# ysymyth/3D-SDN

Hardware: AMD Instinct MI355X
Metric: rendered-objects/sec (FFD decode + transform + silhouette/normal/depth @384, fwd+bwd) (higher is better)
Workload: dtype f32

## Files before the change

3d-sdn_amd/csrc/raster_bwd.hip:

```cpp
#include "raster_math.h"
#include "sdn_common.h"

namespace sdn {

#ifndef SDN_EDGE_CHUNK
#define SDN_EDGE_CHUNK 8
#endif
constexpr int CHUNK = SDN_EDGE_CHUNK;
static_assert(CHUNK == 4 || CHUNK == 8, "k_edge_scan_sil / k_chunk_sum are written for 4 or 8");

struct BwdParams {
    const float* faces;
    const float* textures;
    const float* face_inv;
    const int32_t* face_index_map;
    const float* weight_map;
    const float* depth_map;
    const float* rgb_map;
    const float* g_rgb_out;
    const float* g_alpha_out;
    const float* g_depth_out;
    float* grad_faces;
    float* grad_textures;
    uint32_t* visible;
    int32_t* chunk_base;
    uint32_t* counter;
    uint4* chunk_desc;
    float2* chunk_out;
    const float* hmap;
    const float* hmapT;
    const uint16_t* nz_cnt;
    const uint16_t* nz_pos;
    const float* nz_val;
    uint32_t* row_cnt;
    struct OwnerRec* own_rec;
    float2* own_out;
    uint8_t* chunk_mask;
    uint32_t cap;
    double eps;
    int ts, bs, nf, S, flags;
    VertexSink sink;
};

__host__ __device__ __forceinline__ bool segment_path(const BwdParams& P)
{
#ifdef SDN_LAB_EDGE_PER_FACE
    return false;
#else
    return P.sink.grad_verts != nullptr && P.nz_cnt != nullptr;
#endif
}

struct OwnerRec {
    float t1, t0, cross;
    uint32_t kk;
    uint32_t slot;
};

struct MapReader {
    const BwdParams& P;
    int b, S, R;
    bool aa;
    __device__ MapReader(const BwdParams& p, int bn) : P(p), b(bn), S(p.S)
    {
        aa = (p.flags & SDN_AA) != 0;
        R = aa ? S / 2 : S;
    }
    __device__ __forceinline__ size_t q(int x, int y) const { return ((size_t)b * S + y) * S + x; }
    __device__ __forceinline__ int fidx(int x, int y) const { return P.face_index_map[q(x, y)]; }
    __device__ __forceinline__ float alpha(int x, int y) const { return fidx(x, y) >= 0 ? 1.0f : 0.0f; }
    __device__ __forceinline__ float rgb(int x, int y, int k) const { return P.rgb_map[q(x, y) * 3 + k]; }
    __device__ __forceinline__ size_t oidx(int x, int y) const
    {
        return aa ? ((size_t)((S - 1 - y) >> 1)) * R + (x >> 1) : ((size_t)(S - 1 - y)) * R + x;
    }
    __device__ __forceinline__ float g_alpha(int x, int y) const
    {
        if (!P.g_alpha_out) return 0.0f;
        const float g = P.g_alpha_out[(size_t)b * R * R + oidx(x, y)];
        return aa ? g * 0.25f : g;
    }
    __device__ __forceinline__ float g_depth(int x, int y) const
    {
        if (!P.g_depth_out) return 0.0f;
        const float g = P.g_depth_out[(size_t)b * R * R + oidx(x, y)];
        return aa ? g * 0.25f : g;
    }
    __device__ __forceinline__ float g_rgb(int x, int y, int k) const
    {
        if (!P.g_rgb_out) return 0.0f;
        const float g = P.g_rgb_out[((size_t)b * 3 + k) * R * R + oidx(x, y)];
        return aa ? g * 0.25f : g;
    }
};

__device__ __forceinline__ float edge_dist(float pa, float pb, float denom, int d1, float d1_cross, float is_f,
                                           double eps)
{
    float t = (pb - pa) / denom;
    t = t * ((float)d1 - d1_cross);
    float dist = (2.0f * t) / is_f;
    dist = (0.0f < dist) ? (float)((double)dist + eps) : (float)((double)dist - eps);
    return dist;
}

struct EdgeWalk {
    float p[3][2];
    int pi0, pi1;
    int direction;
    int d0_from, d0_to;
};

__device__ __forceinline__ EdgeWalk edge_walk(const float face[9], int edge_num, int axis, float is_f)
{
    EdgeWalk w;
    int pi[3];
    float pp[3][2];
#pragma unroll
    for (int num = 0; num < 3; num++) {
        pi[num] = (edge_num + num) % 3;
        pp[num][0] = ndc_to_pixel(face[3 * pi[num] + 0], is_f);
        pp[num][1] = ndc_to_pixel(face[3 * pi[num] + 1], is_f);
    }
#pragma unroll
    for (int num = 0; num < 3; num++) {
        w.p[num][0] = pp[num][axis];
        w.p[num][1] = pp[num][1 - axis];
    }
    w.pi0 = pi[0];
    w.pi1 = pi[1];
    if (axis == 0)
        w.direction = (w.p[0][0] < w.p[1][0]) ? -1 : 1;
    else
        w.direction = (w.p[0][0] < w.p[1][0]) ? 1 : -1;
    w.d0_from = cvt_i32(fmaxf(ceilf(fminf(w.p[0][0], w.p[1][0])), 0.0f));
    w.d0_to = cvt_i32(fminf(fmaxf(w.p[0][0], w.p[1][0]), is_f - 1.0f));
    return w;
}

__device__ __forceinline__ void edge_pixel(const BwdParams& P, const MapReader& M, const EdgeWalk& w, int fn, int axis,
                                           int d0, bool use_alpha, bool use_rgb, int lane, int nlanes, float& acc0,
                                           float& acc1)
{
    const int S = P.S;
    const float is_f = (float)S;
    const float fd0 = (float)d0;
    float d1_cross = (w.p[1][1] - w.p[0][1]) / (w.p[1][0] - w.p[0][0]);
    d1_cross = d1_cross * (fd0 - w.p[0][0]);
    d1_cross = d1_cross + w.p[0][1];
    const int d1_in = (0 < w.direction) ? cvt_i32(floorf(d1_cross)) : cvt_i32(ceilf(d1_cross));
    const int d1_out = d1_in + w.direction;
    if (d1_in < 0 || S <= d1_in) return;
    if (d1_out < 0 || S <= d1_out) return;

    const int xin = axis == 0 ? d0 : d1_in, yin = axis == 0 ? d1_in : d0;
    const int xout = axis == 0 ? d0 : d1_out, yout = axis == 0 ? d1_out : d0;
    float alpha_in = 0.f, alpha_out = 0.f, rgb_in[3] = {0, 0, 0}, rgb_out[3] = {0, 0, 0};
    const int f_in = M.fidx(xin, yin);
    if (use_alpha) {
        alpha_in = f_in >= 0 ? 1.0f : 0.0f;
        alpha_out = M.alpha(xout, yout);
    }
    if (use_rgb) {
#pragma unroll
        for (int k = 0; k < 3; k++) {
            rgb_in[k] = M.rgb(xin, yin, k);
            rgb_out[k] = M.rgb(xout, yout, k);
        }
    }
    const bool nz1 = w.p[1][0] != fd0, nz0 = w.p[0][0] != fd0;
    const float den1 = w.p[1][0] - fd0, den0 = fd0 - w.p[0][0];
    const float* hline = nullptr;
    if (P.hmap && use_alpha && !use_rgb) hline = (axis == 0 ? P.hmapT : P.hmap) + ((size_t)M.b * S + d0) * S;

    if (f_in == fn && hline) {
        const int d1_limit = (0 < w.direction) ? S - 1 : 0;
        const int d1_from = max(min(d1_out, d1_limit), 0);
        const int d1_to = min(max(d1_out, d1_limit), S - 1);
        const size_t row = (size_t)(axis == 0 ? P.bs : 0) * S + (size_t)M.b * S + d0;
        const uint16_t* cnt = P.nz_cnt + row * (S + 1);
        const int k1 = cnt[d1_to + 1];
        for (int k = cnt[d1_from] + lane; k < k1; k += nlanes) {
            const int d1 = P.nz_pos[row * S + k];
            const float diff_grad = P.nz_val[row * S + k];
            if (nz1) acc0 -= diff_grad / edge_dist(w.p[0][0], w.p[1][0], den1, d1, d1_cross, is_f, P.eps);
            if (nz0) acc1 -= diff_grad / edge_dist(w.p[0][0], w.p[1][0], den0, d1, d1_cross, is_f, P.eps);
        }
    } else if (f_in == fn) {
        const int d1_limit = (0 < w.direction) ? S - 1 : 0;
        const int d1_from = max(min(d1_out, d1_limit), 0);
        const int d1_to = min(max(d1_out, d1_limit), S - 1);
        for (int d1 = d1_from + lane; d1 <= d1_to; d1 += nlanes) {
            const int x = axis == 0 ? d0 : d1, y = axis == 0 ? d1 : d0;
            float diff_grad = 0.0f;
            if (use_alpha) diff_grad = diff_grad + (M.alpha(x, y) - alpha_in) * M.g_alpha(x, y);
            if (use_rgb) {
#pragma unroll
                for (int k = 0; k < 3; k++) diff_grad = diff_grad + (M.rgb(x, y, k) - rgb_in[k]) * M.g_rgb(x, y, k);
            }
            if (diff_grad <= 0) continue;
            if (nz1) acc0 -= diff_grad / edge_dist(w.p[0][0], w.p[1][0], den1, d1, d1_cross, is_f, P.eps);
            if (nz0) acc1 -= diff_grad / edge_dist(w.p[0][0], w.p[1][0], den0, d1, d1_cross, is_f, P.eps);
        }
    }
    {
        float d0_cross2;
        if ((fd0 - w.p[0][0]) * (fd0 - w.p[2][0]) < 0) {
            d0_cross2 = (w.p[2][1] - w.p[0][1]) / (w.p[2][0] - w.p[0][0]);
            d0_cross2 = d0_cross2 * (fd0 - w.p[0][0]);
            d0_cross2 = d0_cross2 + w.p[0][1];
        } else {
            d0_cross2 = (w.p[1][1] - w.p[2][1]) / (w.p[1][0] - w.p[2][0]);
            d0_cross2 = d0_cross2 * (fd0 - w.p[2][0]);
            d0_cross2 = d0_cross2 + w.p[2][1];
        }
        const int d1_limit = (0 < w.direction) ? cvt_i32(ceilf(d0_cross2)) : cvt_i32(floorf(d0_cross2));
        const int d1_from = max(min(d1_in, d1_limit), 0);
        const int d1_to = min(max(d1_in, d1_limit), S - 1);
        for (int d1 = d1_from + lane; d1 <= d1_to; d1 += nlanes) {
            const int x = axis == 0 ? d0 : d1, y = axis == 0 ? d1 : d0;
            if (M.fidx(x, y) != fn) continue;
            float diff_grad = 0.0f;
            if (use_alpha) diff_grad = diff_grad + (1.0f - alpha_out) * M.g_alpha(x, y);
            if (use_rgb) {
#pragma unroll
                for (int k = 0; k < 3; k++) diff_grad = diff_grad + (M.rgb(x, y, k) - rgb_out[k]) * M.g_rgb(x, y, k);
            }
            if (diff_grad <= 0) continue;
            if (nz1) acc0 -= diff_grad / edge_dist(w.p[0][0], w.p[1][0], den1, d1, d1_cross, is_f, P.eps);
            if (nz0) acc1 -= diff_grad / edge_dist(w.p[0][0], w.p[1][0], den0, d1, d1_cross, is_f, P.eps);
        }
    }
}

__global__ __launch_bounds__(256) void k_mark_visible(const int32_t* __restrict__ face_index_map, long npx, int S,
                                                       int nf, uint32_t* __restrict__ visible)
{
    const long i = (long)blockIdx.x * 256 + threadIdx.x;
    if (i >= npx) return;
    const int fn = face_index_map[i];
    if (fn >= 0) visible[(i / ((long)S * S)) * nf + fn] = 1u;
}

__global__ __launch_bounds__(256) void k_hmap(const BwdParams P, float* __restrict__ hmapT)
{
    __shared__ float tile[32][33];
    const int S = P.S, b = blockIdx.z;
    const MapReader M(P, b);
    const int x = blockIdx.x * 32 + (threadIdx.x & 31);
#pragma unroll
    for (int r = 0; r < 4; r++) {
        const int ly = (threadIdx.x >> 5) + 8 * r, y = blockIdx.y * 32 + ly;
        float h = 0.0f;
        if (x < S && y < S) {
            const int fn = M.fidx(x, y);
            if (fn < 0) {
                const float t = (0.0f - 1.0f) * M.g_alpha(x, y);
                h = t > 0.0f ? t : 0.0f;
            } else {
                P.visible[(size_t)b * P.nf + fn] = 1u;
            }
        }
        tile[ly][threadIdx.x & 31] = h;
    }
    __syncthreads();
    const int yt = blockIdx.y * 32 + (threadIdx.x & 31);
#pragma unroll
    for (int r = 0; r < 4; r++) {
        const int lx = (threadIdx.x >> 5) + 8 * r, xt = blockIdx.x * 32 + lx;
        if (xt < S && yt < S) hmapT[((size_t)b * S + xt) * S + yt] = tile[threadIdx.x & 31][lx];
    }
}

__global__ __launch_bounds__(256) void k_compact_rows(const BwdParams P, const float* __restrict__ mapsT,
                                                      size_t rows_per_map, int S, uint16_t* __restrict__ cnt,
                                                      uint16_t* __restrict__ pos, float* __restrict__ val)
{
    const int lane = threadIdx.x & 63;
    const size_t row = (size_t)blockIdx.x * 4 + (threadIdx.x >> 6);
    if (row >= 2 * rows_per_map) return;
    const bool image_row = row < rows_per_map;
    const float* src = mapsT + (image_row ? 0 : row - rows_per_map) * S;
    const int yb = (int)(row / (size_t)S), yy = (int)(row % (size_t)S);
    const MapReader M(P, image_row ? yb : 0);
    auto h_at = [&](const int x) {
        float h = 0.0f;
        if (M.fidx(x, yy) < 0) {
            const float t = (0.0f - 1.0f) * M.g_alpha(x, yy);
            h = t > 0.0f ? t : 0.0f;
        }
        return h;
    };
    uint16_t* c = cnt + row * (S + 1);
    int base = 0;
    for (int x0 = 0; x0 < S; x0 += 128) {
        const int x = x0 + 2 * lane;
        float h0 = 0.0f, h1 = 0.0f;
        if (image_row) {
            if (x < S) h0 = h_at(x);
            if (x + 1 < S) h1 = h_at(x + 1);
        } else if (x + 1 < S && ((S & 1) == 0)) {
            const float2 v = *reinterpret_cast<const float2*>(src + x);
            h0 = v.x;
            h1 = v.y;
        } else {
            if (x < S) h0 = src[x];
            if (x + 1 < S) h1 = src[x + 1];
        }
        const bool nz0 = h0 > 0.0f, nz1 = h1 > 0.0f;
        const unsigned long long m0 = __ballot(nz0), m1 = __ballot(nz1);
        const unsigned long long below = (1ull << lane) - 1ull;
        const int i0 = base + __popcll(m0 & below) + __popcll(m1 & below);
        const int i1 = i0 + (nz0 ? 1 : 0);
        if (x < S) {
            c[x] = (uint16_t)i0;
            if (nz0) {
                pos[row * S + i0] = (uint16_t)x;
                val[row * S + i0] = h0;
            }
        }
        if (x + 1 < S) {
            c[x + 1] = (uint16_t)i1;
            if (nz1) {
                pos[row * S + i1] = (uint16_t)(x + 1);
                val[row * S + i1] = h1;
            }
        }
        base += __popcll(m0) + __popcll(m1);
    }
    if (lane == 0) c[S] = (uint16_t)base;
}

constexpr int PLAN_THREADS = 1024;
__global__ __launch_bounds__(PLAN_THREADS) void k_edge_plan(const BwdParams P)
{
    const long i = (long)blockIdx.x * PLAN_THREADS + threadIdx.x;
    const long total = (long)P.bs * P.nf;
    if (P.sink.grad_verts) {
        const long n = (long)P.bs * P.sink.nv * 3;
        for (long k = i; k < n; k += (long)gridDim.x * PLAN_THREADS) P.sink.grad_verts[k] = 0.0f;
    }
    const int lane = threadIdx.x & 63;
    int from[6], cnt[6];
    uint32_t nchunks = 0;
    bool contributes = false;
    if (i < total) {
        const bool active = (P.flags & (SDN_ALPHA | SDN_RGB)) != 0;
        if (active && P.visible[i] != 0u) {
            float face[9];
#pragma unroll
            for (int k = 0; k < 9; k++) face[k] = P.faces[i * 9 + k];
            if (!is_backface(face)) {
                const float is_f = (float)P.S;
#pragma unroll
                for (int e = 0; e < 6; e++) {
                    const EdgeWalk w = edge_walk(face, e >> 1, e & 1, is_f);
                    from[e] = w.d0_from;
                    cnt[e] = max(w.d0_to - w.d0_from + 1, 0);
                    nchunks += (uint32_t)((cnt[e] + CHUNK - 1) / CHUNK);
                }
                contributes = nchunks != 0;
            }
        }
    }
    __shared__ uint32_t wave_sum[PLAN_THREADS / 64];
    __shared__ uint32_t block_base;
    uint32_t incl = nchunks;
#pragma unroll
    for (int d = 1; d < 64; d <<= 1) {
        const uint32_t o = __shfl_up(incl, d, 64);
        if (lane >= d) incl += o;
    }
    const int wave = threadIdx.x >> 6;
    if (lane == 63) wave_sum[wave] = incl;
    __syncthreads();
    if (threadIdx.x == 0) {
        uint32_t tot = 0;
        for (int w = 0; w < PLAN_THREADS / 64; w++) tot += wave_sum[w];
        block_base = tot ? atomicAdd(P.counter, tot) : 0u;
    }
    __syncthreads();
    uint32_t wave_base = block_base;
    for (int w = 0; w < wave; w++) wave_base += wave_sum[w];
    if (i >= total) return;
    const bool per_face = !segment_path(P);
    if (!contributes) {
        if (per_face) P.chunk_base[i] = -2;
        return;
    }
    const uint32_t base = wave_base + incl - nchunks;
    if (base + nchunks > P.cap) {
        if (per_face)
            P.chunk_base[i] = -1;
        else
            P.chunk_base[atomicAdd(P.counter + 1, 1u)] = (int32_t)i;
        for (uint32_t c = base; c < P.cap; c++) P.chunk_desc[c] = make_uint4(0xffffffffu, 0xffffffffu, 0u, 0u);
        return;
    }
    if (per_face) P.chunk_base[i] = (int32_t)base;
    uint32_t c = base;
#pragma unroll
    for (int e = 0; e < 6; e++) {
        for (int s = 0; s < cnt[e]; s += CHUNK)
            P.chunk_desc[c++] = make_uint4((uint32_t)i, (uint32_t)e, (uint32_t)(from[e] + s),
                                           (uint32_t)min(CHUNK, cnt[e] - s));
    }
}

__global__ __launch_bounds__(256) void k_edge_scan(const BwdParams P)
{
    const int lane = threadIdx.x & 63;
    const uint32_t wave = (blockIdx.x * 256u + threadIdx.x) >> 6;
    const uint32_t nwaves = (gridDim.x * 256u) >> 6;
    const uint32_t nchunks = min(*P.counter, P.cap);
    const bool use_alpha = (P.flags & SDN_ALPHA) != 0;
    const bool use_rgb = (P.flags & SDN_RGB) != 0;
    const float is_f = (float)P.S;
    for (uint32_t c = wave; c < nchunks; c += nwaves) {
        const uint4 d = P.chunk_desc[c];
        if (d.x >= (uint32_t)((long)P.bs * P.nf)) {
            if (lane == 0) P.chunk_out[c] = make_float2(0.f, 0.f);
            continue;
        }
        const long i = d.x;
        const int bn = (int)(i / P.nf), fn = (int)(i % P.nf);
        float face[9];
#pragma unroll
        for (int k = 0; k < 9; k++) face[k] = P.faces[i * 9 + k];
        const int axis = (int)(d.y & 1u);
        const EdgeWalk w = edge_walk(face, (int)(d.y >> 1), axis, is_f);
        const MapReader M(P, bn);
        float acc0 = 0.f, acc1 = 0.f;
        for (int s = 0; s < (int)d.w; s++)
            edge_pixel(P, M, w, fn, axis, (int)d.z + s, use_alpha, use_rgb, lane, 64, acc0, acc1);
#pragma unroll
        for (int o = 32; o > 0; o >>= 1) {
            acc0 += __shfl_xor(acc0, o, 64);
            acc1 += __shfl_xor(acc1, o, 64);
        }
        if (lane == 0) P.chunk_out[c] = make_float2(acc0, acc1);
    }
}

#ifndef SDN_LAB_IN_LANE_MAX
#define SDN_LAB_IN_LANE_MAX 32
#endif
constexpr int IN_LANE_MAX = SDN_LAB_IN_LANE_MAX;
#ifndef SDN_LAB_COOP_MAX_WALKS
#define SDN_LAB_COOP_MAX_WALKS 32
#endif
constexpr int COOP_MAX_WALKS = SDN_LAB_COOP_MAX_WALKS;

__global__ __launch_bounds__(256) void k_edge_scan_sil(const BwdParams P)
{
    const int lane = threadIdx.x & 63;
    const uint32_t wave = (blockIdx.x * 256u + threadIdx.x) >> 6;
    const uint32_t nwaves = (gridDim.x * 256u) >> 6;
    const uint32_t nchunks = min(*P.counter, P.cap);
    const int S = P.S;
    const float is_f = (float)S;
    const float two_over_is = 2.0f / is_f, eps_f = (float)P.eps;
    const long total_faces = (long)P.bs * P.nf;
    constexpr uint32_t CPW = 64u / CHUNK;
    for (uint32_t c0 = wave * CPW; c0 < nchunks; c0 += nwaves * CPW) {
        const uint32_t c = c0 + (uint32_t)(lane / CHUNK);
        const int s_in = lane % CHUNK;
        float in0 = 0.f, in1 = 0.f;
        int k0 = 0, k1 = 0;
        bool up = false;
        size_t row = 0;
        float pa = 0.f, pb = 0.f, den1 = 1.f, den0 = 1.f, d1_cross = 0.f;
        int nzflags = 0;
        bool chunk_ok = false;
        int w_from = 0, w_to = -1, w_key = 0, w_d0 = 0;
        float w_ta1 = 0.f, w_ta0 = 0.f;
        if (c < nchunks) {
            const uint4 d = P.chunk_desc[c];
            chunk_ok = d.x < (uint32_t)total_faces;
            if (chunk_ok && s_in < (int)d.w) {
                const long i = d.x;
                const int bn = (int)(i / P.nf), fn = (int)(i % P.nf);
                float face[9];
#pragma unroll
                for (int k = 0; k < 9; k++) face[k] = P.faces[i * 9 + k];
                const int axis = (int)(d.y & 1u);
                const EdgeWalk w = edge_walk(face, (int)(d.y >> 1), axis, is_f);
                const MapReader M(P, bn);
                const int d0 = (int)d.z + s_in;
                const float fd0 = (float)d0;
                d1_cross = (w.p[1][1] - w.p[0][1]) / (w.p[1][0] - w.p[0][0]);
                d1_cross = d1_cross * (fd0 - w.p[0][0]);
                d1_cross = d1_cross + w.p[0][1];
                const int d1_in = (0 < w.direction) ? cvt_i32(floorf(d1_cross)) : cvt_i32(ceilf(d1_cross));
                const int d1_out = d1_in + w.direction;
                if (!(d1_in < 0 || S <= d1_in || d1_out < 0 || S <= d1_out)) {
                    const int xin = axis == 0 ? d0 : d1_in, yin = axis == 0 ? d1_in : d0;
                    const int xout = axis == 0 ? d0 : d1_out, yout = axis == 0 ? d1_out : d0;
                    const int f_in = M.fidx(xin, yin);
                    const float alpha_out = M.alpha(xout, yout);
                    const bool nz1 = w.p[1][0] != fd0, nz0 = w.p[0][0] != fd0;
                    pa = w.p[0][0];
                    pb = w.p[1][0];
                    den1 = w.p[1][0] - fd0;
                    den0 = fd0 - w.p[0][0];
                    nzflags = (nz1 ? 1 : 0) | (nz0 ? 2 : 0);
                    if (f_in == fn) {
                        const int d1_limit = (0 < w.direction) ? S - 1 : 0;
                        const int d1_from = max(min(d1_out, d1_limit), 0);
                        const int d1_to = min(max(d1_out, d1_limit), S - 1);
                        row = (size_t)(axis == 0 ? P.bs : 0) * S + (size_t)bn * S + d0;
                        const uint16_t* cnt = P.nz_cnt + row * (S + 1);
                        up = 0 < w.direction;
                        if (up) {
                            k0 = cnt[d1_from];
                            k1 = cnt[S];
                        } else {
                            k0 = 0;
                            k1 = cnt[d1_to + 1];
                        }
                    }
#ifdef SDN_LAB_SCAN_NOIN
                    if (false) {
#else
                    if (alpha_out == 0.0f) {
#endif
                    float d0_cross2;
                    if ((fd0 - w.p[0][0]) * (fd0 - w.p[2][0]) < 0) {
                        d0_cross2 = (w.p[2][1] - w.p[0][1]) / (w.p[2][0] - w.p[0][0]);
                        d0_cross2 = d0_cross2 * (fd0 - w.p[0][0]);
                        d0_cross2 = d0_cross2 + w.p[0][1];
                    } else {
                        d0_cross2 = (w.p[1][1] - w.p[2][1]) / (w.p[1][0] - w.p[2][0]);
                        d0_cross2 = d0_cross2 * (fd0 - w.p[2][0]);
                        d0_cross2 = d0_cross2 + w.p[2][1];
                    }
                    const int d1_limit = (0 < w.direction) ? cvt_i32(ceilf(d0_cross2)) : cvt_i32(floorf(d0_cross2));
                    const int d1_from = max(min(d1_in, d1_limit), 0);
                    const int d1_to = min(max(d1_in, d1_limit), S - 1);
                    const float ta1 = (pb - pa) / den1 * two_over_is, ta0 = (pb - pa) / den0 * two_over_is;
                    w_from = d1_from;
                    w_to = d1_to;
                    w_key = axis | (fn << 1);
                    w_d0 = d0 | (bn << 16);
                    w_ta1 = ta1;
                    w_ta0 = ta0;
                    }
                }
            }
        }
        {
            const bool has = w_to >= w_from;
            unsigned long long lm = __ballot(has && w_to - w_from >= IN_LANE_MAX);
            const bool coop = __popcll(lm) <= COOP_MAX_WALKS;
            if (!coop) lm = 0ull;
            const bool own = has && (coop ? w_to - w_from < IN_LANE_MAX : true);
            while (lm) {
                const int j = __builtin_amdgcn_readfirstlane(__ffsll((long long)lm) - 1);
                lm &= lm - 1ull;
                const int from = __builtin_amdgcn_readlane(w_from, j), to = __builtin_amdgcn_readlane(w_to, j);
                const int key = __builtin_amdgcn_readlane(w_key, j), d0b = __builtin_amdgcn_readlane(w_d0, j);
                const float ta1 = __int_as_float(__builtin_amdgcn_readlane(__float_as_int(w_ta1), j));
                const float ta0 = __int_as_float(__builtin_amdgcn_readlane(__float_as_int(w_ta0), j));
                const float cross = __int_as_float(__builtin_amdgcn_readlane(__float_as_int(d1_cross), j));
                const int nzj = __builtin_amdgcn_readlane(nzflags, j);
                const int axis = key & 1, fn = key >> 1, d0 = d0b & 0xffff;
                const MapReader M(P, d0b >> 16);
                float p0 = 0.f, p1 = 0.f;
                for (int d1 = from + lane; d1 <= to; d1 += 64) {
                    const int x = axis == 0 ? d0 : d1, y = axis == 0 ? d1 : d0;
                    if (M.fidx(x, y) != fn) continue;
                    float diff_grad = 0.0f;
                    diff_grad = diff_grad + (1.0f - 0.0f) * M.g_alpha(x, y);
                    if (diff_grad <= 0) continue;
                    const float dd = (float)d1 - cross;
                    if (nzj & 1) {
                        const float dist = ta1 * dd;
                        p0 -= diff_grad * __builtin_amdgcn_rcpf(0.0f < dist ? dist + eps_f : dist - eps_f);
                    }
                    if (nzj & 2) {
                        const float dist = ta0 * dd;
                        p1 -= diff_grad * __builtin_amdgcn_rcpf(0.0f < dist ? dist + eps_f : dist - eps_f);
                    }
                }
#pragma unroll
                for (int o = 32; o > 0; o >>= 1) {
                    p0 += __shfl_xor(p0, o, 64);
                    p1 += __shfl_xor(p1, o, 64);
                }
                if (lane == j) {
                    in0 += p0;
                    in1 += p1;
                }
            }
            if (own) {
                const int axis = w_key & 1, fn = w_key >> 1, d0 = w_d0 & 0xffff;
                const MapReader M(P, w_d0 >> 16);
                const bool nz1 = (nzflags & 1) != 0, nz0 = (nzflags & 2) != 0;
                for (int d1b = w_from; d1b <= w_to; d1b += 4) {
                    int fi[4];
                    float ga[4];
#pragma unroll
                    for (int u = 0; u < 4; u++) {
                        const int d1 = min(d1b + u, w_to);
                        const int x = axis == 0 ? d0 : d1, y = axis == 0 ? d1 : d0;
                        fi[u] = M.fidx(x, y);
                        ga[u] = M.g_alpha(x, y);
                    }
#pragma unroll
                    for (int u = 0; u < 4; u++) {
                        const int d1 = d1b + u;
                        if (d1 > w_to || fi[u] != fn) continue;
                        float diff_grad = 0.0f;
                        diff_grad = diff_grad + (1.0f - 0.0f) * ga[u];
                        if (diff_grad <= 0) continue;
                        const float dd = (float)d1 - d1_cross;
                        if (nz1) {
                            const float dist = w_ta1 * dd;
                            in0 -= diff_grad * __builtin_amdgcn_rcpf(0.0f < dist ? dist + eps_f : dist - eps_f);
                        }
                        if (nz0) {
                            const float dist = w_ta0 * dd;
                            in1 -= diff_grad * __builtin_amdgcn_rcpf(0.0f < dist ? dist + eps_f : dist - eps_f);
                        }
                    }
                }
            }
        }
#ifdef SDN_LAB_SCAN_NOFILE
        const bool owner = false;
#else
        const bool owner = k1 > k0;
#endif
        if (owner) {
            uint32_t at = atomicAdd(P.row_cnt + 2 * row + (up ? 0 : 1), 1u);
            if (!up) at = (uint32_t)(3 * S) - 1u - at;
            OwnerRec r;
            r.t1 = (pb - pa) / den1 * two_over_is;
            r.t0 = (pb - pa) / den0 * two_over_is;
            r.cross = d1_cross;
            r.kk = (uint32_t)k0 | ((uint32_t)k1 << 16);
            r.slot = (c * (uint32_t)CHUNK + (uint32_t)s_in) | ((uint32_t)nzflags << 30);
            if (at < (uint32_t)(3 * S)) P.own_rec[row * (size_t)(3 * S) + at] = r;
        }
        const unsigned long long owners = __ballot(owner);
        float sum0 = in0, sum1 = in1;
#pragma unroll
        for (int o = CHUNK / 2; o > 0; o >>= 1) {
            const float t0 = __shfl_down(sum0, o, 64), t1 = __shfl_down(sum1, o, 64);
            if (s_in + o < CHUNK) {
                sum0 += t0;
                sum1 += t1;
            }
        }
        if (s_in == 0 && c < nchunks) {
            P.chunk_out[c] = chunk_ok ? make_float2(sum0, sum1) : make_float2(0.f, 0.f);
            P.chunk_mask[c] = chunk_ok ? (uint8_t)((owners >> (lane & ~(CHUNK - 1))) & ((1ull << CHUNK) - 1ull)) : (uint8_t)0;
        }
    }
}

__global__ __launch_bounds__(256) void k_edge_rows(const BwdParams P, int nrows)
{
    extern __shared__ float2 lds_list[];
    const int lane = threadIdx.x & 63, wave = threadIdx.x >> 6;
    const int S = P.S;
    const int row = blockIdx.x;
    const float eps_f = (float)P.eps;
    const uint32_t n_up = min(P.row_cnt[2 * row], (uint32_t)(3 * S));
    const uint32_t n_down = min(P.row_cnt[2 * row + 1], (uint32_t)(3 * S) - n_up);
    if (n_up + n_down == 0) return;
    const int total = P.nz_cnt[(size_t)row * (S + 1) + S];
    for (int k = threadIdx.x; k < total; k += 256)
        lds_list[k] = make_float2((float)P.nz_pos[(size_t)row * S + k], P.nz_val[(size_t)row * S + k]);
    __syncthreads();
    const OwnerRec* recs = P.own_rec + (size_t)row * (3 * S);
    const uint32_t b_up = (n_up + 63) >> 6, b_all = b_up + ((n_down + 63) >> 6);
    for (uint32_t b = wave; b < b_all; b += 4) {
        const bool down = b >= b_up;
        const uint32_t idx = (down ? b - b_up : b) * 64u + lane;
        if (idx >= (down ? n_down : n_up)) continue;
        const OwnerRec r = recs[down ? (uint32_t)(3 * S) - 1u - idx : idx];
        const int k0 = (int)(r.kk & 0xffffu), k1 = (int)(r.kk >> 16);
        const bool nz1 = (r.slot >> 30) & 1u, nz0 = (r.slot >> 31) & 1u;
        typedef float v2f __attribute__((ext_vector_type(2)));
        const v2f t = {r.t1, r.t0};
        const float sdd = down ? -1.0f : 1.0f;
        const v2f es = {0.0f < t.x * sdd ? eps_f : -eps_f, 0.0f < t.y * sdd ? eps_f : -eps_f};
        v2f o[4] = {{0.f, 0.f}, {0.f, 0.f}, {0.f, 0.f}, {0.f, 0.f}};
        auto term = [&](const float2 e, v2f& a) {
            float val = e.y;
#ifndef SDN_LAB_ROWS_HI_SPLAT
            asm volatile("" : "+v"(val));
#endif
            const float dd = e.x - r.cross;
            v2f dist = t * dd;
#ifdef SDN_LAB_ROWS_EPS_PER_ENTRY
            const v2f s = {0.0f < dist.x ? eps_f : -eps_f, 0.0f < dist.y ? eps_f : -eps_f};
            dist = dist + s;
#else
            dist = dist + es;
#endif
            const v2f rc = {__builtin_amdgcn_rcpf(dist.x), __builtin_amdgcn_rcpf(dist.y)};
            a = a - val * rc;
        };
        int k = k0;
        for (; k + 4 <= k1; k += 4) {
            const float2 e0 = lds_list[k], e1 = lds_list[k + 1], e2 = lds_list[k + 2], e3 = lds_list[k + 3];
            term(e0, o[0]);
            term(e1, o[1]);
            term(e2, o[2]);
            term(e3, o[3]);
        }
        if (k < k1) term(lds_list[k], o[0]);
        if (k + 1 < k1) term(lds_list[k + 1], o[1]);
        if (k + 2 < k1) term(lds_list[k + 2], o[2]);
        const v2f sum = (o[0] + o[1]) + (o[2] + o[3]);
        P.own_out[r.slot & 0x3fffffffu] = make_float2(nz1 ? sum.x : 0.0f, nz0 ? sum.y : 0.0f);
    }
}

__device__ __forceinline__ float2 chunk_add_owners(const BwdParams& P, uint32_t c, uint32_t m, float2 a)
{
    const float4* q = reinterpret_cast<const float4*>(P.own_out + (size_t)c * CHUNK);
#pragma unroll
    for (int h = 0; h < CHUNK / 2; h++) {
        if (!(m & (3u << (2 * h)))) continue;
        const float4 v = q[h];
        if (m & (1u << (2 * h))) {
            a.x += v.x;
            a.y += v.y;
        }
        if (m & (2u << (2 * h))) {
            a.x += v.z;
            a.y += v.w;
        }
    }
    return a;
}

__global__ __launch_bounds__(256) void k_chunk_sum(const BwdParams P)
{
    const uint32_t nchunks = min(*P.counter, P.cap);
    const uint32_t c = blockIdx.x * 256u + threadIdx.x;
    if (c >= nchunks) return;
    uint32_t m = P.chunk_mask[c];
    if (!m) return;
    P.chunk_out[c] = chunk_add_owners(P, c, m, P.chunk_out[c]);
}

__device__ __forceinline__ void sink_add_face(const BwdParams& P, long i, const float grad_face[9])
{
    bool any = false;
#pragma unroll
    for (int k = 0; k < 9; k++) any = any || grad_face[k] != 0.0f;
    if (!any) return;
    const int bn = (int)(i / P.nf), fn = (int)(i % P.nf);
    const bool twin = P.sink.fill_back && fn >= P.sink.nf0;
    const int32_t* idx = P.sink.faces_idx + (size_t)bn * P.sink.fstride + (size_t)(twin ? fn - P.sink.nf0 : fn) * 3;
#pragma unroll
    for (int k = 0; k < 3; k++) {
        float* dst = P.sink.grad_verts + ((size_t)bn * P.sink.nv + idx[twin ? 2 - k : k]) * 3;
#pragma unroll
        for (int d = 0; d < 3; d++)
            if (grad_face[3 * k + d] != 0.0f) unsafeAtomicAdd(&dst[d], grad_face[3 * k + d]);
    }
}

__global__ __launch_bounds__(256) void k_edge_reduce(const BwdParams P)
{
    const long i = (long)blockIdx.x * 256 + threadIdx.x;
    const long total = (long)P.bs * P.nf;
    if (i >= total) return;
    const bool accumulate = (P.flags & SDN_ACCUMULATE) != 0;
    if ((P.flags & SDN_SPARSE_GRAD) && P.visible[i] == 0u) return;
    const int32_t base = P.chunk_base[i];
    float grad_face[9] = {0, 0, 0, 0, 0, 0, 0, 0, 0};
    if (base != -2) {
        float face[9];
#pragma unroll
        for (int k = 0; k < 9; k++) face[k] = P.faces[i * 9 + k];
        const float is_f = (float)P.S;
        const bool use_alpha = (P.flags & SDN_ALPHA) != 0;
        const bool use_rgb = (P.flags & SDN_RGB) != 0;
        const int bn = (int)(i / P.nf), fn = (int)(i % P.nf);
        uint32_t c = (uint32_t)base;
        for (int e = 0; e < 6; e++) {
            const int axis = e & 1;
            const EdgeWalk w = edge_walk(face, e >> 1, axis, is_f);
            float a0 = 0.f, a1 = 0.f;
            if (base >= 0) {
                const int cnt = max(w.d0_to - w.d0_from + 1, 0);
                const int nch = (cnt + CHUNK - 1) / CHUNK;
                for (int s = 0; s < nch; s += 8) {
                    float2 o[8];
#pragma unroll
                    for (int u = 0; u < 8; u++)
                        if (s + u < nch) o[u] = P.chunk_out[c + s + u];
#pragma unroll
                    for (int u = 0; u < 8; u++)
                        if (s + u < nch) {
                            a0 += o[u].x;
                            a1 += o[u].y;
                        }
                }
                c += (uint32_t)nch;
                grad_face[w.pi0 * 3 + (1 - axis)] += a0;
                grad_face[w.pi1 * 3 + (1 - axis)] += a1;
            } else {
                const MapReader M(P, bn);
                for (int d0 = w.d0_from; d0 <= w.d0_to; d0++)
                    edge_pixel(P, M, w, fn, axis, d0, use_alpha, use_rgb, 0, 1, grad_face[w.pi0 * 3 + (1 - axis)],
                               grad_face[w.pi1 * 3 + (1 - axis)]);
            }
        }
    }
    if (P.sink.grad_verts) {
        if (base == -2) return;
        sink_add_face(P, i, grad_face);
        return;
    }
    if (accumulate) {
#pragma unroll
        for (int k = 0; k < 9; k++) P.grad_faces[i * 9 + k] += grad_face[k];
    } else {
#pragma unroll
        for (int k = 0; k < 9; k++) P.grad_faces[i * 9 + k] = grad_face[k];
    }
}

constexpr int SEG_SERIAL_BLOCKS = 8;

__device__ __forceinline__ void segment_add(const BwdParams& P, long i, int e, float a0, float a1)
{
    if (a0 == 0.0f && a1 == 0.0f) return;
    const int bn = (int)(i / P.nf), fn = (int)(i % P.nf);
    const int axis = e & 1, pi0 = e >> 1, pi1 = (pi0 + 1) % 3;
    const bool twin = P.sink.fill_back && fn >= P.sink.nf0;
    const int32_t* idx = P.sink.faces_idx + (size_t)bn * P.sink.fstride + (size_t)(twin ? fn - P.sink.nf0 : fn) * 3;
    float* g = P.sink.grad_verts + (size_t)bn * P.sink.nv * 3 + (1 - axis);
    if (a0 != 0.0f) unsafeAtomicAdd(&g[(size_t)idx[twin ? 2 - pi0 : pi0] * 3], a0);
    if (a1 != 0.0f) unsafeAtomicAdd(&g[(size_t)idx[twin ? 2 - pi1 : pi1] * 3], a1);
}

__global__ __launch_bounds__(256) void k_edge_segments(const BwdParams P)
{
    const int lane = threadIdx.x & 63;
    if (blockIdx.x < SEG_SERIAL_BLOCKS) {
        const uint32_t n = P.counter[1];
        constexpr uint32_t WAVES = SEG_SERIAL_BLOCKS * 4;
        const uint32_t wave = blockIdx.x * 4u + (threadIdx.x >> 6);
        const bool use_alpha = (P.flags & SDN_ALPHA) != 0, use_rgb = (P.flags & SDN_RGB) != 0;
        const float is_f = (float)P.S;
        for (uint32_t k = (uint32_t)lane * WAVES + wave; k < n; k += 64u * WAVES) {
            const long i = P.chunk_base[k];
            const int bn = (int)(i / P.nf), fn = (int)(i % P.nf);
            float face[9];
#pragma unroll
            for (int j = 0; j < 9; j++) face[j] = P.faces[i * 9 + j];
            const MapReader M(P, bn);
            float grad_face[9] = {0, 0, 0, 0, 0, 0, 0, 0, 0};
            for (int e = 0; e < 6; e++) {
                const int axis = e & 1;
                const EdgeWalk w = edge_walk(face, e >> 1, axis, is_f);
                for (int d0 = w.d0_from; d0 <= w.d0_to; d0++)
                    edge_pixel(P, M, w, fn, axis, d0, use_alpha, use_rgb, 0, 1, grad_face[w.pi0 * 3 + (1 - axis)],
                               grad_face[w.pi1 * 3 + (1 - axis)]);
            }
            sink_add_face(P, i, grad_face);
        }
        return;
    }
    const uint32_t nchunks = min(*P.counter, P.cap);
    const uint32_t c = (blockIdx.x - (uint32_t)SEG_SERIAL_BLOCKS) * 256u + threadIdx.x;
    const uint32_t c_wave = (uint32_t)__builtin_amdgcn_readfirstlane((int)(c - (uint32_t)lane));
    if (c_wave >= nchunks) return;
    const uint32_t total = (uint32_t)((long)P.bs * P.nf);
    auto key_at = [&](uint32_t s) { return *reinterpret_cast<const uint2*>(P.chunk_desc + s); };
    uint2 d = make_uint2(0xffffffffu, 0xffffffffu);
    float2 v = make_float2(0.f, 0.f);
    uint32_t m = 0u;
    if (c < nchunks) {
        d = key_at(c);
        v = P.chunk_out[c];
        m = P.chunk_mask[c];
    }
    uint2 before = make_uint2(0xffffffffu, 0xffffffffu), after = before;
    if (c_wave > 0u) before = key_at(c_wave - 1u);
    if (c_wave + 64u < nchunks) after = key_at(c_wave + 64u);
    const bool valid = d.x < total;
    if (valid && m) v = chunk_add_owners(P, c, m, v);
    uint32_t px = __shfl_up(d.x, 1, 64), py = __shfl_up(d.y, 1, 64);
    if (lane == 0) {
        px = before.x;
        py = before.y;
    }
    const bool head = valid && (px != d.x || py != d.y);
    const unsigned long long bounds = __ballot(head || !valid);
    const unsigned long long above = lane == 63 ? 0ull : bounds >> (lane + 1);
    const int len = head ? (above ? __ffsll((long long)above) : 64 - lane) : 0;
    float a0 = 0.f, a1 = 0.f;
    for (int k = 0; __ballot(k < len) != 0ull; k++) {
        const float tx = __shfl(v.x, lane + k, 64), ty = __shfl(v.y, lane + k, 64);
        if (k < len) {
            a0 += tx;
            a1 += ty;
        }
    }
    const unsigned long long runs_on = __ballot(head && !above && after.x == d.x && after.y == d.y);
    if (runs_on) {
        const int hl = __ffsll((long long)runs_on) - 1;
        const uint32_t kx = (uint32_t)__builtin_amdgcn_readlane((int)d.x, hl), ky = (uint32_t)__builtin_amdgcn_readlane((int)d.y, hl);
        for (uint32_t s0 = c_wave + 64u; s0 < nchunks; s0 += 64u) {
            const uint32_t s = s0 + (uint32_t)lane;
            uint2 ds = make_uint2(0xffffffffu, 0xffffffffu);
            float2 vs = make_float2(0.f, 0.f);
            uint32_t ms = 0u;
            if (s < nchunks) {
                ds = key_at(s);
                vs = P.chunk_out[s];
                ms = P.chunk_mask[s];
            }
            const bool mine = ds.x == kx && ds.y == ky;
            if (mine && ms) vs = chunk_add_owners(P, s, ms, vs);
            const unsigned long long others = ~__ballot(mine);
            const int n = others ? __ffsll((long long)others) - 1 : 64;
            for (int k = 0; k < n; k++) {
                const float tx = __shfl(vs.x, k, 64), ty = __shfl(vs.y, k, 64);
                if (lane == hl) {
                    a0 += tx;
                    a1 += ty;
                }
            }
            if (n < 64) break;
        }
    }
    if (!head) return;
    segment_add(P, (long)d.x, (int)d.y, a0, a1);
}

__global__ __launch_bounds__(256) void k_bwd_pixels(const BwdParams P)
{
    const long i = (long)blockIdx.x * 256 + threadIdx.x;
    const long npx = (long)P.bs * P.S * P.S;
    if (i >= npx) return;
    const int fn = P.face_index_map[i];
    if (fn < 0) return;
    const int S = P.S;
    const int bn = (int)(i / ((long)S * S));
    const int pn = (int)(i % ((long)S * S));
    const int yi = pn / S, xi = pn % S;
    const MapReader M(P, bn);
    const size_t fidx = (size_t)bn * P.nf + fn;
    float face[9];
#pragma unroll
    for (int k = 0; k < 9; k++) face[k] = P.faces[fidx * 9 + k];
    const float depth = P.depth_map[i];
    const float w[3] = {P.weight_map[i * 3 + 0], P.weight_map[i * 3 + 1], P.weight_map[i * 3 + 2]};

    if ((P.flags & SDN_DEPTH) && P.g_depth_out) {
        float inv[9];
#pragma unroll
        for (int k = 0; k < 9; k++) inv[k] = P.face_inv[fidx * 9 + k];
        const float g = M.g_depth(xi, yi);
        const float depth2 = depth * depth;
        float* gf = P.grad_faces + fidx * 9;
#pragma unroll
        for (int k = 0; k < 3; k++) {
            const float zk = face[3 * k + 2];
            float t = g * w[k];
            t = t * depth2;
            t = t / (zk * zk);
            unsafeAtomicAdd(&gf[3 * k + 2], t);
        }
        float tmp[2] = {0.f, 0.f};
#pragma unroll
        for (int k = 0; k < 2; k++)
#pragma unroll
            for (int l = 0; l < 3; l++) tmp[k] = tmp[k] + (-inv[3 * l + k] / face[3 * l + 2]);
#pragma unroll
        for (int k = 0; k < 3; k++)
#pragma unroll
            for (int l = 0; l < 2; l++) {
                float t = -g * tmp[l];
                t = t * w[k];
                t = t * depth2;
                t = t * (float)S;
                t = t / 2.0f;
                unsafeAtomicAdd(&gf[3 * k + l], t);
            }
    }
    if ((P.flags & SDN_RGB) && P.g_rgb_out && P.grad_textures) {
        const bool face_color = (P.flags & SDN_FACE_COLOR) != 0;
        const int ts = face_color ? 2 : P.ts;
        const TexCoord tc = texture_coord(w, depth, face[2], face[5], face[8], ts, P.eps);
        const float g[3] = {M.g_rgb(xi, yi, 0), M.g_rgb(xi, yi, 1), M.g_rgb(xi, yi, 2)};
        if (face_color) {
            float acc[3] = {0.f, 0.f, 0.f};
#pragma unroll
            for (int c = 0; c < 8; c++) {
                int isc;
                float wgt;
                texture_corner(tc, c, ts, isc, wgt);
#pragma unroll
                for (int k = 0; k < 3; k++) acc[k] = acc[k] + wgt * g[k];
            }
#pragma unroll
            for (int k = 0; k < 3; k++) unsafeAtomicAdd(&P.grad_textures[fidx * 3 + k], acc[k]);
        } else {
            float* gt = P.grad_textures + fidx * (size_t)ts * ts * ts * 3;
#pragma unroll
            for (int c = 0; c < 8; c++) {
                int isc;
                float wgt;
                texture_corner(tc, c, ts, isc, wgt);
#pragma unroll
                for (int k = 0; k < 3; k++) unsafeAtomicAdd(&gt[(long)isc * 3 + k], wgt * g[k]);
            }
        }
    }
}

}

using namespace sdn;

static size_t align256(size_t n) { return (n + 255) & ~(size_t)255; }

static void bwd_layout(int bs, int nf, int S, size_t off[14], uint32_t& cap, size_t& total)
{
    const size_t n = (size_t)bs * nf;
    cap = (uint32_t)(4 * n + 65536);
    off[0] = 0;
    off[1] = 256;
    off[10] = off[1] + align256(n * sizeof(uint32_t));
    off[2] = off[10] + align256((size_t)4 * bs * S * sizeof(uint32_t));
    off[3] = off[2] + align256(n * sizeof(int32_t));
    off[4] = off[3] + align256((size_t)cap * sizeof(uint4));
    off[5] = off[4] + align256((size_t)cap * sizeof(float2));
    off[6] = off[5];
    off[7] = off[6] + align256((size_t)bs * S * S * sizeof(float));
    off[8] = off[7] + align256((size_t)2 * bs * S * (S + 1) * sizeof(uint16_t));
    off[9] = off[8] + align256((size_t)2 * bs * S * S * sizeof(uint16_t));
    off[11] = off[9] + align256((size_t)2 * bs * S * S * sizeof(float));
    off[12] = off[11] + align256((size_t)2 * bs * S * 3 * S * sizeof(OwnerRec));
    off[13] = off[12] + align256((size_t)cap * 8 * sizeof(float2));
    total = off[13] + align256((size_t)cap);
}

namespace sdn {
const uint32_t* raster_bwd_visible_flags(const void* workspace) { return (const uint32_t*)((const char*)workspace + 256); }
}

SDN_API int sdn_raster_bwd_workspace_bytes(int bs, int nf, int S, size_t* out)
{
    if (bs <= 0 || nf <= 0 || S <= 0 || !out) return fail(SDN_EINVAL, "sdn_raster_bwd_workspace_bytes: bad sizes");
    size_t off[14], total;
    uint32_t cap;
    bwd_layout(bs, nf, S, off, cap, total);
    *out = total;
    return SDN_OK;
}

SDN_API int sdn_rasterize_bwd(const float* faces, const float* textures, int ts, int bs, int nf, int S, double eps,
                              int flags, const float* face_inv, const int32_t* face_index_map,
                              const float* weight_map, const float* depth_map, const float* rgb_map,
                              const float* g_rgb_out, const float* g_alpha_out, const float* g_depth_out,
                              float* grad_faces, float* grad_textures, void* workspace, size_t workspace_bytes,
                              sdnStream stream)
{
    return rasterize_bwd_core(nullptr, faces, textures, ts, bs, nf, S, eps, flags, face_inv, face_index_map, weight_map, depth_map,
                              rgb_map, g_rgb_out, g_alpha_out, g_depth_out, grad_faces, grad_textures, workspace, workspace_bytes,
                              stream);
}

int sdn::rasterize_bwd_core(const VertexSink* sink, const float* faces, const float* textures, int ts, int bs, int nf, int S,
                            double eps, int flags, const float* face_inv, const int32_t* face_index_map, const float* weight_map,
                            const float* depth_map, const float* rgb_map, const float* g_rgb_out, const float* g_alpha_out,
                            const float* g_depth_out, float* grad_faces, float* grad_textures, void* workspace,
                            size_t workspace_bytes, sdnStream stream)
{
    if (!faces || !face_inv || !face_index_map || !weight_map || !depth_map || (!grad_faces && !sink) || bs <= 0 || nf <= 0 ||
        S <= 0)
        return fail(SDN_EINVAL, "sdn_rasterize_bwd: missing state (was the forward run with SDN_SAVE_MAPS?)");
    if (sink && ((flags & (SDN_RGB | SDN_DEPTH | SDN_ACCUMULATE)) || !(flags & SDN_ALPHA) || !g_alpha_out || !sink->faces_idx ||
                 !sink->grad_verts || nf != (sink->fill_back ? 2 : 1) * sink->nf0))
        return fail(SDN_EINVAL, "rasterize_bwd_core: the vertex sink takes a silhouette-only pass");
    if ((flags & SDN_RGB) && (!rgb_map || !textures))
        return fail(SDN_EINVAL, "sdn_rasterize_bwd: rgb gradients need rgb_map and textures");
    if ((flags & SDN_AA) && (S & 1)) return fail(SDN_EINVAL, "sdn_rasterize_bwd: SDN_AA needs an even internal size");
    size_t off[14], need;
    uint32_t cap;
    bwd_layout(bs, nf, S, off, cap, need);
    if (!workspace || workspace_bytes < need)
        return fail(SDN_ENOMEM, "sdn_rasterize_bwd: workspace %zu < %zu bytes", workspace_bytes, need);
    hipStream_t st = (hipStream_t)stream;
    BwdParams P;
    P.faces = faces;
    P.textures = textures;
    P.face_inv = face_inv;
    P.face_index_map = face_index_map;
    P.weight_map = weight_map;
    P.depth_map = depth_map;
    P.rgb_map = rgb_map;
    P.g_rgb_out = (flags & SDN_RGB) ? g_rgb_out : nullptr;
    P.g_alpha_out = (flags & SDN_ALPHA) ? g_alpha_out : nullptr;
    P.g_depth_out = (flags & SDN_DEPTH) ? g_depth_out : nullptr;
    P.grad_faces = grad_faces;
    P.grad_textures = grad_textures;
    char* ws = (char*)workspace;
    P.counter = (uint32_t*)(ws + off[0]);
    P.visible = (uint32_t*)(ws + off[1]);
    P.chunk_base = (int32_t*)(ws + off[2]);
    P.chunk_desc = (uint4*)(ws + off[3]);
    P.chunk_out = (float2*)(ws + off[4]);
    P.hmap = nullptr;
    P.hmapT = nullptr;
    P.nz_cnt = nullptr;
    P.nz_pos = nullptr;
    P.nz_val = nullptr;
    P.row_cnt = nullptr;
    P.own_rec = nullptr;
    P.own_out = nullptr;
    P.chunk_mask = nullptr;
    P.cap = (flags & SDN_SERIAL_EDGES) ? 0u : cap;
    P.eps = eps;
    P.ts = ts;
    P.bs = bs;
    P.nf = nf;
    P.S = S;
    P.flags = flags;
    P.sink = sink ? *sink : VertexSink{nullptr, 0, 0, 0, 0, nullptr};
    if (!P.g_rgb_out) P.flags &= ~SDN_RGB;
    if (!P.g_alpha_out) P.flags &= ~SDN_ALPHA;
    const long total = (long)bs * nf;
    const long npx = (long)bs * S * S;
    const bool edges = (P.flags & (SDN_ALPHA | SDN_RGB)) != 0;
    if (!edges) P.flags &= ~SDN_SPARSE_GRAD;
    int rc;
    if (edges) {
        hipError_t e = hipMemsetAsync(ws, 0, off[2], st);
        if (e != hipSuccess) return fail(SDN_ELAUNCH, "hipMemsetAsync(plan): %s", hipGetErrorString(e));
        const bool sil_path = (P.flags & SDN_ALPHA) && !(P.flags & SDN_RGB) && !(flags & SDN_SERIAL_EDGES);
        if (!sil_path) {
            hipLaunchKernelGGL(k_mark_visible, dim3(cdiv(npx, 256)), dim3(256), 0, st, face_index_map, npx, S, nf,
                               P.visible);
            if ((rc = check_launch("k_mark_visible"))) return rc;
        }
        if (sil_path) {
            float* hmap = (float*)(ws + off[5]);
            float* hmapT = (float*)(ws + off[6]);
            if (S > 65535) return fail(SDN_EINVAL, "sdn_rasterize_bwd: internal size %d exceeds the 16-bit row index", S);
            uint16_t* cnt = (uint16_t*)(ws + off[7]);
            uint16_t* pos = (uint16_t*)(ws + off[8]);
            float* val = (float*)(ws + off[9]);
            const size_t rows = (size_t)bs * S;
            hipLaunchKernelGGL(k_hmap, dim3(cdiv(S, 32), cdiv(S, 32), bs), dim3(256), 0, st, P, hmapT);
            if ((rc = check_launch("k_hmap"))) return rc;
            hipLaunchKernelGGL(k_compact_rows, dim3((unsigned)cdiv((long)(2 * rows), 4)), dim3(256), 0, st, P, hmapT, rows, S, cnt, pos,
                               val);
            if ((rc = check_launch("k_compact_rows"))) return rc;
            P.hmap = hmap;
            P.hmapT = hmapT;
            P.nz_cnt = cnt;
            P.nz_pos = pos;
            P.nz_val = val;
            if ((size_t)cap * 8 >= (1u << 30)) return fail(SDN_EINVAL, "sdn_rasterize_bwd: %u chunks exceed the 30-bit slot index", cap);
            P.row_cnt = (uint32_t*)(ws + off[10]);
            P.own_rec = (OwnerRec*)(ws + off[11]);
            P.own_out = (float2*)(ws + off[12]);
            P.chunk_mask = (uint8_t*)(ws + off[13]);
        }
    }
    hipLaunchKernelGGL(k_edge_plan, dim3(cdiv(total, PLAN_THREADS)), dim3(PLAN_THREADS), 0, st, P);
    if ((rc = check_launch("k_edge_plan"))) return rc;
    if (edges) {
        {
            TimedLaunch timed(TIME_EDGE_SCAN, st, 0.0);
            if (P.nz_cnt) {
                hipLaunchKernelGGL(k_edge_scan_sil, dim3(256 * 8), dim3(256), 0, st, P);
                const int nrows = 2 * bs * S;
                hipLaunchKernelGGL(k_edge_rows, dim3((unsigned)nrows), dim3(256), (size_t)S * sizeof(float2), st, P, nrows);
                if (!segment_path(P)) hipLaunchKernelGGL(k_chunk_sum, dim3(cdiv((long)cap, 256)), dim3(256), 0, st, P);
            } else
                hipLaunchKernelGGL(k_edge_scan, dim3(256 * 8), dim3(256), 0, st, P);
        }
        if ((rc = check_launch("k_edge_scan"))) return rc;
    }
    if (segment_path(P)) {
        hipLaunchKernelGGL(k_edge_segments, dim3((unsigned)(cdiv((long)cap, 256) + SEG_SERIAL_BLOCKS)), dim3(256), 0, st, P);
        if ((rc = check_launch("k_edge_segments"))) return rc;
    } else {
        hipLaunchKernelGGL(k_edge_reduce, dim3(cdiv(total, 256)), dim3(256), 0, st, P);
        if ((rc = check_launch("k_edge_reduce"))) return rc;
    }

    const bool need_tex = (P.flags & SDN_RGB) && grad_textures;
    if (need_tex && !(flags & SDN_ACCUMULATE)) {
        const size_t n = (flags & SDN_FACE_COLOR) ? (size_t)total * 3 : (size_t)total * ts * ts * ts * 3;
        hipError_t e = hipMemsetAsync(grad_textures, 0, n * sizeof(float), st);
        if (e != hipSuccess) return fail(SDN_ELAUNCH, "hipMemsetAsync(grad_textures): %s", hipGetErrorString(e));
    }
    if (((P.flags & SDN_DEPTH) && P.g_depth_out) || need_tex) {
        hipLaunchKernelGGL(k_bwd_pixels, dim3(cdiv(npx, 256)), dim3(256), 0, st, P);
        if ((rc = check_launch("k_bwd_pixels"))) return rc;
    }
    return SDN_OK;
}
```

Before: 24550.

## Replace float hit maps with coverage bitmasks and low-res gradient transpose

```diff
diff --git a/3d-sdn_amd/csrc/raster_bwd.hip b/3d-sdn_amd/csrc/raster_bwd.hip
--- a/3d-sdn_amd/csrc/raster_bwd.hip
+++ b/3d-sdn_amd/csrc/raster_bwd.hip
@@ -27,8 +27,6 @@
     uint32_t* counter;
     uint4* chunk_desc;
     float2* chunk_out;
-    const float* hmap;
-    const float* hmapT;
     const uint16_t* nz_cnt;
     const uint16_t* nz_pos;
     const float* nz_val;
@@ -170,10 +168,9 @@
     }
     const bool nz1 = w.p[1][0] != fd0, nz0 = w.p[0][0] != fd0;
     const float den1 = w.p[1][0] - fd0, den0 = fd0 - w.p[0][0];
-    const float* hline = nullptr;
-    if (P.hmap && use_alpha && !use_rgb) hline = (axis == 0 ? P.hmapT : P.hmap) + ((size_t)M.b * S + d0) * S;
-
-    if (f_in == fn && hline) {
+    const bool sparse_rows = P.nz_cnt && use_alpha && !use_rgb;
+
+    if (f_in == fn && sparse_rows) {
         const int d1_limit = (0 < w.direction) ? S - 1 : 0;
         const int d1_from = max(min(d1_out, d1_limit), 0);
         const int d1_to = min(max(d1_out, d1_limit), S - 1);
@@ -242,37 +239,52 @@
     if (fn >= 0) visible[(i / ((long)S * S)) * nf + fn] = 1u;
 }
 
-__global__ __launch_bounds__(256) void k_hmap(const BwdParams P, float* __restrict__ hmapT)
-{
-    __shared__ float tile[32][33];
-    const int S = P.S, b = blockIdx.z;
-    const MapReader M(P, b);
-    const int x = blockIdx.x * 32 + (threadIdx.x & 31);
+__global__ __launch_bounds__(256) void k_cover_bits(const BwdParams P, uint32_t* __restrict__ cov, uint32_t* __restrict__ covT,
+                                                    float* __restrict__ gT)
+{
+    __shared__ uint32_t flag[32][33];
+    __shared__ float gt[32][33];
+    const int S = P.S, b = blockIdx.z, W = (S + 31) >> 5;
+    const bool aa = (P.flags & SDN_AA) != 0;
+    const int R = aa ? S / 2 : S, n = aa ? 16 : 32;
+    const int lx = threadIdx.x & 31, l8 = threadIdx.x >> 5;
+    const unsigned half = threadIdx.x & 32;
+    const int x = blockIdx.x * 32 + lx;
+    int fn[4];
+    float gv[4];
 #pragma unroll
     for (int r = 0; r < 4; r++) {
-        const int ly = (threadIdx.x >> 5) + 8 * r, y = blockIdx.y * 32 + ly;
-        float h = 0.0f;
-        if (x < S && y < S) {
-            const int fn = M.fidx(x, y);
-            if (fn < 0) {
-                const float t = (0.0f - 1.0f) * M.g_alpha(x, y);
-                h = t > 0.0f ? t : 0.0f;
-            } else {
-                P.visible[(size_t)b * P.nf + fn] = 1u;
-            }
-        }
-        tile[ly][threadIdx.x & 31] = h;
+        const int ly = l8 + 8 * r, y = blockIdx.y * 32 + ly;
+        const int xo = blockIdx.x * n + lx, yo = blockIdx.y * n + ly;
+        fn[r] = (x < S && y < S) ? P.face_index_map[((size_t)b * S + y) * S + x] : -1;
+        gv[r] = (lx < n && ly < n && xo < R && yo < R) ? P.g_alpha_out[((size_t)b * R + yo) * R + xo] : 0.0f;
+    }
+#pragma unroll
+    for (int r = 0; r < 4; r++) {
+        const int ly = l8 + 8 * r, y = blockIdx.y * 32 + ly;
+        const bool covered = fn[r] >= 0;
+        const int left = __shfl_up(fn[r], 1);
+        if (covered && ((threadIdx.x & 63) == 0 || left != fn[r])) P.visible[(size_t)b * P.nf + fn[r]] = 1u;
+        flag[ly][lx] = covered ? 1u : 0u;
+        gt[ly][lx] = gv[r];
+        const unsigned long long m = __ballot(covered);
+        if (lx == 0 && y < S) cov[((size_t)b * S + y) * W + blockIdx.x] = (uint32_t)(m >> half);
     }
     __syncthreads();
-    const int yt = blockIdx.y * 32 + (threadIdx.x & 31);
 #pragma unroll
     for (int r = 0; r < 4; r++) {
-        const int lx = (threadIdx.x >> 5) + 8 * r, xt = blockIdx.x * 32 + lx;
-        if (xt < S && yt < S) hmapT[((size_t)b * S + xt) * S + yt] = tile[threadIdx.x & 31][lx];
-    }
-}
-
-__global__ __launch_bounds__(256) void k_compact_rows(const BwdParams P, const float* __restrict__ mapsT,
+        const int lc = l8 + 8 * r, xt = blockIdx.x * 32 + lc;
+        const unsigned long long m = __ballot(flag[lx][lc] != 0u);
+        if (lx == 0 && xt < S) covT[((size_t)b * S + xt) * W + blockIdx.y] = (uint32_t)(m >> half);
+        const int xo = blockIdx.x * n + lc, yo = blockIdx.y * n + lx;
+        if (lx < n && lc < n && xo < R && yo < R) gT[((size_t)b * R + xo) * R + yo] = gt[lx][lc];
+    }
+}
+
+constexpr int CR = 6;
+template <bool AA>
+__global__ __launch_bounds__(256) void k_compact_rows(const BwdParams P, const uint32_t* __restrict__ cov,
+                                                      const uint32_t* __restrict__ covT, const float* __restrict__ gT,
                                                       size_t rows_per_map, int S, uint16_t* __restrict__ cnt,
                                                       uint16_t* __restrict__ pos, float* __restrict__ val)
 {
@@ -280,55 +292,75 @@
     const size_t row = (size_t)blockIdx.x * 4 + (threadIdx.x >> 6);
     if (row >= 2 * rows_per_map) return;
     const bool image_row = row < rows_per_map;
-    const float* src = mapsT + (image_row ? 0 : row - rows_per_map) * S;
-    const int yb = (int)(row / (size_t)S), yy = (int)(row % (size_t)S);
-    const MapReader M(P, image_row ? yb : 0);
-    auto h_at = [&](const int x) {
-        float h = 0.0f;
-        if (M.fidx(x, yy) < 0) {
-            const float t = (0.0f - 1.0f) * M.g_alpha(x, yy);
-            h = t > 0.0f ? t : 0.0f;
-        }
-        return h;
-    };
+    const size_t line = image_row ? row : row - rows_per_map;
+    const int b = (int)(line / (size_t)S), d0 = (int)(line % (size_t)S);
+    const int R = AA ? S / 2 : S, W = (S + 31) >> 5;
+    const uint32_t* cw = (image_row ? cov : covT) + line * W;
+    const float* gl = image_row ? P.g_alpha_out + ((size_t)b * R + (R - 1 - (AA ? d0 >> 1 : d0))) * R
+                                : gT + ((size_t)b * R + (AA ? d0 >> 1 : d0)) * R;
     uint16_t* c = cnt + row * (S + 1);
+    const bool odd = ((row * (size_t)(S + 1)) & 1) != 0;
+    const unsigned long long below = (1ull << lane) - 1ull;
     int base = 0;
-    for (int x0 = 0; x0 < S; x0 += 128) {
-        const int x = x0 + 2 * lane;
-        float h0 = 0.0f, h1 = 0.0f;
-        if (image_row) {
-            if (x < S) h0 = h_at(x);
-            if (x + 1 < S) h1 = h_at(x + 1);
-        } else if (x + 1 < S && ((S & 1) == 0)) {
-            const float2 v = *reinterpret_cast<const float2*>(src + x);
-            h0 = v.x;
-            h1 = v.y;
-        } else {
-            if (x < S) h0 = src[x];
-            if (x + 1 < S) h1 = src[x + 1];
-        }
-        const bool nz0 = h0 > 0.0f, nz1 = h1 > 0.0f;
-        const unsigned long long m0 = __ballot(nz0), m1 = __ballot(nz1);
-        const unsigned long long below = (1ull << lane) - 1ull;
-        const int i0 = base + __popcll(m0 & below) + __popcll(m1 & below);
-        const int i1 = i0 + (nz0 ? 1 : 0);
-        if (x < S) {
-            c[x] = (uint16_t)i0;
-            if (nz0) {
-                pos[row * S + i0] = (uint16_t)x;
-                val[row * S + i0] = h0;
-            }
-        }
-        if (x + 1 < S) {
-            c[x + 1] = (uint16_t)i1;
-            if (nz1) {
-                pos[row * S + i1] = (uint16_t)(x + 1);
-                val[row * S + i1] = h1;
-            }
-        }
-        base += __popcll(m0) + __popcll(m1);
-    }
-    if (lane == 0) c[S] = (uint16_t)base;
+    if (AA && odd && lane == 0) c[0] = 0;
+    for (int e0 = 0; e0 < R; e0 += 64 * CR) {
+        float g[CR];
+        uint32_t w[CR];
+#pragma unroll
+        for (int j = 0; j < CR; j++) {
+            const int e = e0 + 64 * j + lane;
+            g[j] = 0.0f;
+            w[j] = 0u;
+            if (e < R) {
+                g[j] = gl[image_row ? e : R - 1 - e];
+                w[j] = cw[AA ? e >> 4 : e >> 5];
+            }
+        }
+#pragma unroll
+        for (int j = 0; j < CR; j++) {
+            const int e = e0 + 64 * j + lane;
+            if (e0 + 64 * j >= R) break;
+            const float t = (0.0f - 1.0f) * (AA ? g[j] * 0.25f : g[j]);
+            const float h = t > 0.0f ? t : 0.0f;
+            const bool in = e < R && h > 0.0f;
+            if (AA) {
+                const uint32_t two = w[j] >> (2 * (e & 15));
+                const bool nz0 = in && !(two & 1u), nz1 = in && !(two & 2u);
+                const unsigned long long m0 = __ballot(nz0), m1 = __ballot(nz1);
+                const int i0 = base + __popcll(m0 & below) + __popcll(m1 & below);
+                const int i1 = i0 + (nz0 ? 1 : 0), i2 = i1 + (nz1 ? 1 : 0);
+                if (e < R) {
+                    const int x = 2 * e;
+                    if (odd)
+                        *reinterpret_cast<uint32_t*>(c + x + 1) = (uint32_t)i1 | (uint32_t)i2 << 16;
+                    else
+                        *reinterpret_cast<uint32_t*>(c + x) = (uint32_t)i0 | (uint32_t)i1 << 16;
+                    if (nz0) {
+                        pos[row * S + i0] = (uint16_t)x;
+                        val[row * S + i0] = h;
+                    }
+                    if (nz1) {
+                        pos[row * S + i1] = (uint16_t)(x + 1);
+                        val[row * S + i1] = h;
+                    }
+                }
+                base += __popcll(m0) + __popcll(m1);
+            } else {
+                const bool nz = in && !((w[j] >> (e & 31)) & 1u);
+                const unsigned long long m = __ballot(nz);
+                const int i0 = base + __popcll(m & below);
+                if (e < R) {
+                    c[e] = (uint16_t)i0;
+                    if (nz) {
+                        pos[row * S + i0] = (uint16_t)e;
+                        val[row * S + i0] = h;
+                    }
+                }
+                base += __popcll(m);
+            }
+        }
+    }
+    if (lane == 0 && !(AA && odd)) c[S] = (uint16_t)base;
 }
 
 constexpr int PLAN_THREADS = 1024;
@@ -1113,8 +1145,6 @@
     P.chunk_base = (int32_t*)(ws + off[2]);
     P.chunk_desc = (uint4*)(ws + off[3]);
     P.chunk_out = (float2*)(ws + off[4]);
-    P.hmap = nullptr;
-    P.hmapT = nullptr;
     P.nz_cnt = nullptr;
     P.nz_pos = nullptr;
     P.nz_val = nullptr;
@@ -1140,27 +1170,33 @@
     if (edges) {
         hipError_t e = hipMemsetAsync(ws, 0, off[2], st);
         if (e != hipSuccess) return fail(SDN_ELAUNCH, "hipMemsetAsync(plan): %s", hipGetErrorString(e));
-        const bool sil_path = (P.flags & SDN_ALPHA) && !(P.flags & SDN_RGB) && !(flags & SDN_SERIAL_EDGES);
+        const size_t cov_words = (size_t)(S + 31) / 32;
+        const bool setup_fits = 2 * (size_t)bs * S * cov_words * sizeof(uint32_t) <= off[7] - off[6] &&
+                                (size_t)bs * S * S * sizeof(float) <= off[12] - off[11];
+        const bool sil_path = (P.flags & SDN_ALPHA) && !(P.flags & SDN_RGB) && !(flags & SDN_SERIAL_EDGES) && setup_fits;
         if (!sil_path) {
             hipLaunchKernelGGL(k_mark_visible, dim3(cdiv(npx, 256)), dim3(256), 0, st, face_index_map, npx, S, nf,
                                P.visible);
             if ((rc = check_launch("k_mark_visible"))) return rc;
         }
         if (sil_path) {
-            float* hmap = (float*)(ws + off[5]);
-            float* hmapT = (float*)(ws + off[6]);
             if (S > 65535) return fail(SDN_EINVAL, "sdn_rasterize_bwd: internal size %d exceeds the 16-bit row index", S);
+            const bool aa = (P.flags & SDN_AA) != 0;
+            const size_t rows = (size_t)bs * S;
+            uint32_t* cov = (uint32_t*)(ws + off[6]);
+            uint32_t* covT = cov + rows * cov_words;
+            float* gT = (float*)(ws + off[11]);
             uint16_t* cnt = (uint16_t*)(ws + off[7]);
             uint16_t* pos = (uint16_t*)(ws + off[8]);
             float* val = (float*)(ws + off[9]);
-            const size_t rows = (size_t)bs * S;
-            hipLaunchKernelGGL(k_hmap, dim3(cdiv(S, 32), cdiv(S, 32), bs), dim3(256), 0, st, P, hmapT);
-            if ((rc = check_launch("k_hmap"))) return rc;
-            hipLaunchKernelGGL(k_compact_rows, dim3((unsigned)cdiv((long)(2 * rows), 4)), dim3(256), 0, st, P, hmapT, rows, S, cnt, pos,
-                               val);
+            hipLaunchKernelGGL(k_cover_bits, dim3(cdiv(S, 32), cdiv(S, 32), bs), dim3(256), 0, st, P, cov, covT, gT);
+            if ((rc = check_launch("k_cover_bits"))) return rc;
+            const dim3 grid((unsigned)cdiv((long)(2 * rows), 4));
+            if (aa)
+                hipLaunchKernelGGL(k_compact_rows<true>, grid, dim3(256), 0, st, P, cov, covT, gT, rows, S, cnt, pos, val);
+            else
+                hipLaunchKernelGGL(k_compact_rows<false>, grid, dim3(256), 0, st, P, cov, covT, gT, rows, S, cnt, pos, val);
             if ((rc = check_launch("k_compact_rows"))) return rc;
-            P.hmap = hmap;
-            P.hmapT = hmapT;
             P.nz_cnt = cnt;
             P.nz_pos = pos;
             P.nz_val = val;
```

Result: faster. 25020 (median of 6 runs) (+1.9%).
